# robotic-vision-lab/Learning-Implicitly-From-Spatial-Transformers-Network

Measured on AMD Instinct MI355X. Metric: SDF query-points/sec (B=8, N=20k, 224^2), higher is better.
Workload: dtype fp16

## Files before the change

learning-implicitly-from-spatial-transformers-network_amd/csrc/prep_kernels.hip:

```cpp
#include "list_common.h"
#include "gather_math.h"

namespace list {

constexpr int kResizeCg = 32;
constexpr int kResizeMaxMs = 320;

__global__ __launch_bounds__(256) void k_prep_img(ListMap2D m, int ms, int Ct, int coff, int f16,
                                                  void* __restrict__ out) {
  __shared__ float tile[kResizeMaxMs * (kResizeCg + 1)];
  const int b = blockIdx.x / ms;
  const int y = blockIdx.x - b * ms;
  const int c0 = blockIdx.y * kResizeCg;
  const int nc = min(kResizeCg, m.C - c0);

  const float sy = ms > 1 ? (float)(m.H - 1) / (float)(ms - 1) : 0.f;
  const float sx = ms > 1 ? (float)(m.W - 1) / (float)(ms - 1) : 0.f;
  const float fy = sy * (float)y;
  const int y0 = min((int)fy, m.H - 1);
  const int y1 = y0 + (y0 < m.H - 1 ? 1 : 0);
  const float wy1 = fy - (float)y0, wy0 = 1.f - wy1;
  const float* base = m.data + (int64_t)b * m.sb;

  for (int idx = threadIdx.x; idx < nc * ms; idx += 256) {
    const int cl = idx / ms;
    const int x = idx - cl * ms;
    const float fx = sx * (float)x;
    const int x0 = min((int)fx, m.W - 1);
    const int x1 = x0 + (x0 < m.W - 1 ? 1 : 0);
    const float wx1 = fx - (float)x0, wx0 = 1.f - wx1;
    const float* pc = base + (int64_t)(c0 + cl) * m.sc;
    const float v00 = pc[(int64_t)y0 * m.sh + (int64_t)x0 * m.sw];
// ... 457 lines not shown
    const uint2 lo = half4(make_float4(v[0], v[1], v[2], v[3])), hi = half4(make_float4(v[4], v[5], v[6], v[7]));
    *(uint4*)((unsigned short*)out + o) = make_uint4(lo.x, lo.y, hi.x, hi.y);
  } else {
    *(float4*)((float*)out + o) = make_float4(v[0], v[1], v[2], v[3]);
    *(float4*)((float*)out + o + 4) = make_float4(v[4], v[5], v[6], v[7]);
  }
}

hipError_t launch_img_level_rows(const ListMap2D* maps, void* const* outs, int n, int B, int f16, hipStream_t s) {
  if (n < 1 || n > LIST_N_IMG_LEVELS || B < 1) return hipErrorInvalidValue;
  LevelRowsArgs a;
  a.n = n; a.B = B;
  int64_t blocks = 0;
  for (int i = 0; i < n; ++i) {
    const ListMap2D& m = maps[i];
    if (m.C % 64 || m.H < 1 || m.W < 1) return hipErrorInvalidValue;
    a.m[i] = m; a.out[i] = outs[i]; a.blk_begin[i] = (int)blocks;
    blocks += (int64_t)B * ((m.H * m.W + 31) / 32) * (m.C / 64);
    if (blocks >= 2147483647LL) return hipErrorInvalidValue;
  }
  for (int i = n; i < LIST_N_IMG_LEVELS; ++i) { a.m[i] = maps[0]; a.out[i] = outs[0]; a.blk_begin[i] = (int)blocks; }
  a.blk_begin[LIST_N_IMG_LEVELS] = (int)blocks;
  if (f16) hipLaunchKernelGGL(k_img_level_rows<1>, dim3((unsigned)blocks), dim3(256), 0, s, a);
  else hipLaunchKernelGGL(k_img_level_rows<0>, dim3((unsigned)blocks), dim3(256), 0, s, a);
  return hipGetLastError();
}

constexpr int kProjPx = 64, kProjN = 256;
struct ProjLevelArgs {
  ListMap2D m[LIST_N_IMG_LEVELS]; const unsigned short* w[LIST_N_IMG_LEVELS]; unsigned short* out[LIST_N_IMG_LEVELS];
  int blk_begin[LIST_N_IMG_LEVELS + 1]; int n, B, H1, ldw;
};

__global__ __launch_bounds__(256) void k_proj_level_nchw(ProjLevelArgs a) {
  __shared__ uint4 As[2][kProjPx * 8];
  int r = 0;
#pragma unroll
  for (int i = 1; i < LIST_N_IMG_LEVELS; ++i)
    if (i < a.n && (int)blockIdx.x >= a.blk_begin[i]) r = i;
  const int l = a.n - 1 - r;
  const ListMap2D m = a.m[l];
  const int npx = m.H * m.W, pbs = (npx + kProjPx - 1) / kProjPx, nts = a.H1 / kProjN;
  int idx = (int)blockIdx.x - a.blk_begin[r];
  const int nt = idx % nts; idx /= nts;
  const int pb = idx % pbs;
  const int b = idx / pbs;
  const int p0 = pb * kProjPx, n0 = nt * kProjN;
  const int lane = threadIdx.x & 63, wave = threadIdx.x >> 6;
  const int col = lane & 15, ko = lane >> 4;
  const int px = min(p0 + lane, npx - 1);
  const int y = px / m.W, x = px - y * m.W;
  const float* src = m.data + (int64_t)b * m.sb + (int64_t)y * m.sh + (int64_t)x * m.sw + (int64_t)(16 * wave) * m.sc;
  const unsigned short* wrow = a.w[l] + (int64_t)(n0 + wave * 64 + col) * a.ldw + 8 * ko;
  const int nk = m.C / 64;
  float v[16];
  auto fetch = [&](int t) {
#pragma unroll
    for (int k = 0; k < 16; ++k) v[k] = src[(int64_t)(t * 64 + k) * m.sc];
  };
  f32x4v acc[4][4];
#pragma unroll
  for (int i = 0; i < 4; ++i)
#pragma unroll
    for (int j = 0; j < 4; ++j) acc[i][j] = (f32x4v){0.f, 0.f, 0.f, 0.f};
  f16x8 bw[2][4], bn[2][4];
  auto fetch_w = [&](int t, f16x8 (&d)[2][4]) {
#pragma unroll
    for (int ks = 0; ks < 2; ++ks)
#pragma unroll
      for (int j = 0; j < 4; ++j) d[ks][j] = *(const f16x8*)(wrow + (int64_t)(j * 16) * a.ldw + t * 64 + ks * 32);
  };
  fetch(0);
  fetch_w(0, bw);
#pragma unroll 1
  for (int t = 0; t < nk; ++t) {
    uint4* buf = As[t & 1];
#pragma unroll
    for (int o = 0; o < 2; ++o) {
      const uint2 lo = half4(make_float4(v[8 * o], v[8 * o + 1], v[8 * o + 2], v[8 * o + 3]));
      const uint2 hi = half4(make_float4(v[8 * o + 4], v[8 * o + 5], v[8 * o + 6], v[8 * o + 7]));
      buf[lane * 8 + ((2 * wave + o) ^ (lane & 7))] = make_uint4(lo.x, lo.y, hi.x, hi.y);
    }
    if (t + 1 < nk) { fetch(t + 1); fetch_w(t + 1, bn); }
    __syncthreads();
#pragma unroll
    for (int ks = 0; ks < 2; ++ks) {
      f16x8 fa[4];
#pragma unroll
      for (int i = 0; i < 4; ++i)
        fa[i] = __builtin_bit_cast(f16x8, buf[(i * 16 + col) * 8 + ((4 * ks + ko) ^ (col & 7))]);
#pragma unroll
      for (int i = 0; i < 4; ++i)
#pragma unroll
        for (int j = 0; j < 4; ++j) acc[i][j] = __builtin_amdgcn_mfma_f32_16x16x32_f16(bw[ks][j], fa[i], acc[i][j], 0, 0, 0);
    }
#pragma unroll
    for (int ks = 0; ks < 2; ++ks)
#pragma unroll
      for (int j = 0; j < 4; ++j) bw[ks][j] = bn[ks][j];
  }
#pragma unroll
  for (int i = 0; i < 4; ++i) {
    const int p = p0 + i * 16 + col;
    if (p >= npx) continue;
    unsigned short* o = a.out[l] + ((int64_t)b * npx + p) * a.H1 + n0 + wave * 64 + 4 * ko;
#pragma unroll
    for (int j = 0; j < 4; ++j)
      *(uint2*)(o + j * 16) = half4(make_float4(acc[i][j][0], acc[i][j][1], acc[i][j][2], acc[i][j][3]));
  }
}

hipError_t launch_proj_levels_nchw(const ListMap2D* maps, const void* const* w, void* const* outs, int n, int B, int H1,
                                   int ldw, hipStream_t s, int order) {
  if (n < 1 || n > LIST_N_IMG_LEVELS || B < 1 || H1 < kProjN || H1 % kProjN || ldw < 64 || ldw % 8) return hipErrorInvalidValue;
  ProjLevelArgs a;
  a.n = n; a.B = B; a.H1 = H1; a.ldw = ldw;
  int64_t blocks = 0;
  for (int r = 0; r < n; ++r) {
    const int i = n - 1 - r;
    const ListMap2D& m = maps[i];
    if (m.C < 64 || m.C % 64 || m.H < 1 || m.W < 1 || (reinterpret_cast<uintptr_t>(w[i]) & 15) ||
        (reinterpret_cast<uintptr_t>(outs[i]) & 7))
      return hipErrorInvalidValue;
    a.m[i] = m; a.w[i] = (const unsigned short*)w[i]; a.out[i] = (unsigned short*)outs[i]; a.blk_begin[r] = (int)blocks;
    blocks += (int64_t)B * ((m.H * m.W + kProjPx - 1) / kProjPx) * (H1 / kProjN);
    if (blocks >= 2147483647LL) return hipErrorInvalidValue;
  }
  for (int i = n; i < LIST_N_IMG_LEVELS; ++i) { a.m[i] = a.m[0]; a.w[i] = a.w[0]; a.out[i] = a.out[0]; a.blk_begin[i] = (int)blocks; }
  a.blk_begin[LIST_N_IMG_LEVELS] = (int)blocks;
  LIST_LAUNCH(k_proj_level_nchw, dim3((unsigned)blocks), dim3(256), 0, s, order, a);
  return hipGetLastError();
}

constexpr int kProjMaxSrc = LIST_N_IMG_LEVELS;
struct ProjSumArgs { ListMap2D src[kProjMaxSrc]; int n_src, B, ms, Ct, coff, H1, RY, nyt, nxt; };

template <int F16, int NL, int SRC16>
__global__ __launch_bounds__(kRowsPx * 8) void k_proj_resize_sum(ProjSumArgs a, void* __restrict__ out) {
  const int bid = xcd_contiguous_block(blockIdx.x, gridDim.x);
  const int cgroups = a.H1 / kRowsCg;
  int idx = bid;
  const int xt = idx % a.nxt; idx /= a.nxt;
  const int cg = idx % cgroups; idx /= cgroups;
  const int yt = idx % a.nyt;
  const int b = idx / a.nyt;
  const int ms = a.ms;
  const int q = threadIdx.x & 7, xi = threadIdx.x >> 3;
  const int xo = xt * kRowsPx + xi;
  const bool active = xo < ms;
  const int x = active ? xo : ms - 1;
  const int c = cg * kRowsCg + 8 * q;

  float top[NL][8], bot[NL][8];
  int row_top[NL], row_bot[NL];
  int64_t p0[NL], p1[NL];
// ... 40 lines not shown
    for (int k = 0; k < 8; ++k) o[k] = 0.f;
#pragma unroll
    for (int l = 0; l < NL; ++l) {
      const int H = a.src[l].H;
      const float fy = sy[l] * (float)y;
      const int y0 = min((int)fy, H - 1);
      const int y1 = y0 + (y0 < H - 1 ? 1 : 0);
      const float wy1 = fy - (float)y0, wy0 = 1.f - wy1;
      if (y0 != row_top[l]) {
        if (y0 == row_bot[l]) {
#pragma unroll
          for (int k = 0; k < 8; ++k) top[l][k] = bot[l][k];
        } else {
          hrow(l, y0, top[l]);
        }
        row_top[l] = y0;
      }
      if (y1 != row_bot[l]) {
        if (y1 == row_top[l]) {
#pragma unroll
          for (int k = 0; k < 8; ++k) bot[l][k] = top[l][k];
        } else {
          hrow(l, y1, bot[l]);
        }
        row_bot[l] = y1;
      }
#pragma unroll
      for (int k = 0; k < 8; ++k) o[k] += top[l][k] * wy0 + bot[l][k] * wy1;
    }
    if (!active) continue;
    if (F16) {
      const uint2 lo = half4(make_float4(o[0], o[1], o[2], o[3]));
      const uint2 hi = half4(make_float4(o[4], o[5], o[6], o[7]));
      *(uint4*)((unsigned short*)out + oi) = make_uint4(lo.x, lo.y, hi.x, hi.y);
    } else {
      *(float4*)((float*)out + oi) = make_float4(o[0], o[1], o[2], o[3]);
      *(float4*)((float*)out + oi + 4) = make_float4(o[4], o[5], o[6], o[7]);
    }
  }
}

hipError_t launch_proj_resize_sum(const ListMap2D* src, int n_src, int B, int map_size, int Ct, int coff, int f16,
                                  void* out, hipStream_t s, int src_f16) {
  if (n_src < 1 || n_src > kProjMaxSrc || map_size < 2 || B < 1) return hipErrorInvalidValue;
  ProjSumArgs a;
  a.n_src = n_src; a.B = B; a.ms = map_size; a.Ct = Ct; a.coff = coff; a.H1 = src[0].C;
  if (a.H1 % kRowsCg || coff % 8 || Ct % 8) return hipErrorInvalidValue;
  float sy_max = 0.f;
  for (int l = 0; l < n_src; ++l) {
    const ListMap2D& m = src[l];
    const int al = src_f16 ? 8 : 4;
    if (m.C != a.H1 || m.sc != 1 || (m.sw % al) || (m.sh % al) || (m.sb % al) || (reinterpret_cast<uintptr_t>(m.data) & 15))
      return hipErrorInvalidValue;
    a.src[l] = m;
    const float sy = (float)(m.H - 1) / (float)(map_size - 1);
    sy_max = sy > sy_max ? sy : sy_max;
  }
  for (int l = n_src; l < kProjMaxSrc; ++l) a.src[l] = src[0];
  int ry = (int)(6.6f / (sy_max > 0.05f ? sy_max : 0.05f) + 0.5f);
  a.RY = ry < 2 ? 2 : (ry > kRowsRyMax ? kRowsRyMax : ry);
  a.nyt = (map_size + a.RY - 1) / a.RY;
  a.nxt = (map_size + kRowsPx - 1) / kRowsPx;
  const int64_t wgs = (int64_t)B * a.nyt * (a.H1 / kRowsCg) * a.nxt;
  if (wgs <= 0 || wgs >= 2147483647LL) return hipErrorInvalidValue;
  const dim3 grid((unsigned)wgs), block(kRowsPx * 8);
#define LIST_PROJ_SUM(NL)                                                                      \
  case NL:                                                                                     \
// ... 304 lines not shown
```

learning-implicitly-from-spatial-transformers-network_amd/csrc/gemm_kernels.hip:

```cpp
#include <type_traits>

#include "list_common.h"
#include "mfma_common.h"
#include "point_math.h"
#include "gather_math.h"

namespace list {

constexpr int BM = 256, BN = 256;
constexpr int kLdsBytes = 131072;
constexpr int kProjRecBytes = BM * (int)sizeof(RowProjRec);

template <int TERMS> struct Pipe {
  static constexpr int kPlanes = TERMS == 3 ? 4 : 2;
  static constexpr int BK = TERMS == 3 ? 32 : 64;
  static constexpr int kRowBytes = BK * 2;
  static constexpr int kPlaneBytes = BM * kRowBytes;
  static constexpr int kStageBytes = kPlanes * kPlaneBytes;
  static constexpr int kStages = kLdsBytes / kStageBytes;
  static constexpr int kAhead = kStages - 1;
  static constexpr int kRowsPerPiece = 1024 / kRowBytes;
  static constexpr int kPiecesPerWave = BM / kRowsPerPiece / 8;
  static constexpr int kLoadsPerStage = kPiecesPerWave * kPlanes;
  static constexpr int kWOff = (TERMS == 3 ? 2 : 1) * kPlaneBytes;
  __device__ static __forceinline__ int swz(int row) {
    return kRowBytes == 64 ? ((row >> 2) & 3) : ((row >> 1) & 7);
  }
};

template <int TERMS>
__device__ __forceinline__ void stage_tiles(const GemmParams& p, char* sbase, int m0, int n0,
                                            int kbyte, int wave, int lane) {
// ... 726 lines not shown
        ah[i] = *(const bf16x8*)(cur + a_row_off + i * 16 * P::kRowBytes + coff);
        if (TERMS == 3)
          al[i] = *(const bf16x8*)(cur + P::kPlaneBytes + a_row_off + i * 16 * P::kRowBytes + coff);
      }
#pragma unroll
      for (int j = 0; j < 4; ++j) {
        wh[j] = *(const bf16x8*)(cur + P::kWOff + w_row_off + j * 16 * P::kRowBytes + coff);
        if (TERMS == 3)
          wl[j] = *(const bf16x8*)(cur + P::kWOff + P::kPlaneBytes + w_row_off + j * 16 * P::kRowBytes + coff);
      }
#pragma unroll
      for (int i = 0; i < 8; ++i)
#pragma unroll
        for (int j = 0; j < 4; ++j) {
          if (TERMS == 3) {
            acc[i][j] = mfma16<0>(al[i], wh[j], acc[i][j]);
            acc[i][j] = mfma16<0>(ah[i], wl[j], acc[i][j]);
          }
          acc[i][j] = mfma16<FP16>(ah[i], wh[j], acc[i][j]);
        }
    }
  }

  gemm_epilogue16<EPI, FP16>(p, acc, smem, m0, n0, wm, wn, wave, lane);
}

struct TailParams {
  GemmParams fc1;
  const char* w2; const float* b2;
  const float* w3; const float* b3; float* sdf; const int* order; int n_valid;
};
constexpr int kTailLds = 163840;

__global__ __launch_bounds__(512, 2) void k_mlp_tail_f16(TailParams tp) {
  using P = Pipe<1>;
  __shared__ __attribute__((aligned(16))) char smem[kTailLds];
  const int lane = threadIdx.x & 63;
  const int wave = __builtin_amdgcn_readfirstlane(threadIdx.x >> 6);
  const int m0 = xcd_contiguous_block(blockIdx.x, gridDim.x) * BM;
  const int col = lane & 15, q = lane >> 4;
  const int fswz = P::swz(col);
  const GemmParams& p = tp.fc1;

  auto w2_base = [&](int kt) -> char* { return smem + (kt == 0 ? 131072 : (kt - 1) * 32768); };
  auto stage_w2 = [&](int kt) {
#pragma unroll
    for (int r = 0; r < 4; ++r) {
      const int piece = 4 * wave + r;
      const int row = piece * 8 + lane / 8;
      const int chunk = (lane % 8) ^ P::swz(row);
      glds16(tp.w2 + (int64_t)row * 512 + kt * 128 + chunk * 16, w2_base(kt) + piece * 1024);
    }
  };
  stage_w2(0);

  f32x4v acc[16][2];
#pragma unroll
  for (int i = 0; i < 16; ++i)
#pragma unroll
    for (int j = 0; j < 2; ++j)
#pragma unroll
      for (int e = 0; e < 4; ++e) acc[i][j][e] = 0.f;
  const int h_row_off = (wave * 32 + col) * P::kRowBytes;
  const int wrow_e = 8 * (col >> 2) + (col & 3), wrow_o = wrow_e + 4;
  const int wswz_e = P::swz(wrow_e), wswz_o = P::swz(wrow_o);
  const int nk = p.K / P::BK;
  stage_tiles<1>(p, smem, m0, 0, 0, wave, lane);
  for (int t = 0; t < nk; ++t) {
    wait_vmcnt<0>();
    __builtin_amdgcn_s_barrier();
    if (t + 1 < nk) stage_tiles<1>(p, smem + ((t + 1) & 1) * P::kStageBytes, m0, 0, (t + 1) * P::kRowBytes, wave, lane);
    const char* cur = smem + (t & 1) * P::kStageBytes;
#pragma unroll
    for (int s2 = 0; s2 < 2; ++s2) {
      const int coff = ((4 * s2 + q) ^ fswz) << 4;
      bf16x8 hf[2];
#pragma unroll
      for (int rt = 0; rt < 2; ++rt) hf[rt] = *(const bf16x8*)(cur + h_row_off + rt * 16 * P::kRowBytes + coff);
#pragma unroll
      for (int nt = 0; nt < 16; ++nt) {
        const int wrow = 32 * (nt >> 1) + ((nt & 1) ? wrow_o : wrow_e);
        const bf16x8 wf = *(const bf16x8*)(cur + P::kWOff + wrow * P::kRowBytes + (((4 * s2 + q) ^ ((nt & 1) ? wswz_o : wswz_e)) << 4));
#pragma unroll
        for (int rt = 0; rt < 2; ++rt) acc[nt][rt] = mfma16<1>(wf, hf[rt], acc[nt][rt]);
      }
    }
  }
  float4 b1v[16];
#pragma unroll
  for (int nt = 0; nt < 16; ++nt) b1v[nt] = *(const float4*)(p.bias + 32 * (nt >> 1) + 8 * q + 4 * (nt & 1));
  __syncthreads();
  stage_w2(1); stage_w2(2); stage_w2(3);
  uint2 h2[16][2];
#pragma unroll
  for (int nt = 0; nt < 16; ++nt) {
    const float bb[4] = {b1v[nt].x, b1v[nt].y, b1v[nt].z, b1v[nt].w};
#pragma unroll
    for (int rt = 0; rt < 2; ++rt) {
      float v[4];
#pragma unroll
      for (int e = 0; e < 4; ++e) v[e] = relu_nan(acc[nt][rt][e] + bb[e]);
      h2[nt][rt] = make_uint2(f2h2(v[0], v[1]), f2h2(v[2], v[3]));
    }
  }
  f32x4v acc2[16][2];
#pragma unroll
  for (int i = 0; i < 16; ++i)
#pragma unroll
    for (int j = 0; j < 2; ++j)
#pragma unroll
      for (int e = 0; e < 4; ++e) acc2[i][j][e] = 0.f;
#pragma unroll
  for (int ks = 0; ks < 8; ++ks) {
    if (ks == 2) { wait_vmcnt<8>(); __builtin_amdgcn_s_barrier(); }
    if (ks == 4) { wait_vmcnt<4>(); __builtin_amdgcn_s_barrier(); }
    if (ks == 6) { wait_vmcnt<0>(); __builtin_amdgcn_s_barrier(); }
    const char* wt = w2_base(ks >> 1);
    const int coff = ((4 * (ks & 1) + q) ^ fswz) << 4;
    bf16x8 hb[2];
#pragma unroll
    for (int rt = 0; rt < 2; ++rt)
      hb[rt] = __builtin_bit_cast(bf16x8, make_uint4(h2[2 * ks][rt].x, h2[2 * ks][rt].y, h2[2 * ks + 1][rt].x, h2[2 * ks + 1][rt].y));
#pragma unroll
    for (int mt = 0; mt < 16; ++mt) {
      const bf16x8 wf = *(const bf16x8*)(wt + (mt * 16 + col) * P::kRowBytes + coff);
#pragma unroll
      for (int rt = 0; rt < 2; ++rt) acc2[mt][rt] = mfma16<1>(wf, hb[rt], acc2[mt][rt]);
    }
  }
  float grp[2][4];
#pragma unroll
  for (int gq = 0; gq < 4; ++gq) {
    float sc[2][4];
#pragma unroll
    for (int rt = 0; rt < 2; ++rt)
#pragma unroll
      for (int e = 0; e < 4; ++e) sc[rt][e] = 0.f;
#pragma unroll
    for (int j = 0; j < 4; ++j) {
      const int mt = 4 * gq + j;
      const float4 b2v = *(const float4*)(tp.b2 + 16 * mt + 4 * q), w3v = *(const float4*)(tp.w3 + 16 * mt + 4 * q);
      const float bb[4] = {b2v.x, b2v.y, b2v.z, b2v.w}, ww[4] = {w3v.x, w3v.y, w3v.z, w3v.w};
#pragma unroll
      for (int rt = 0; rt < 2; ++rt)
#pragma unroll
        for (int e = 0; e < 4; ++e) sc[rt][e] += relu_nan(acc2[mt][rt][e] + bb[e]) * ww[e];
    }
#pragma unroll
    for (int rt = 0; rt < 2; ++rt) {
#pragma unroll
      for (int e = 0; e < 4; ++e) {
        sc[rt][e] += __shfl_xor(sc[rt][e], 32);
        sc[rt][e] += __shfl_xor(sc[rt][e], 16);
      }
      const float a0 = sc[rt][0] + sc[rt][2], a1 = sc[rt][1] + sc[rt][3];
      grp[rt][gq] = a0 + a1;
    }
  }
#pragma unroll
  for (int rt = 0; rt < 2; ++rt) {
    const int row = m0 + wave * 32 + rt * 16 + col;
    if (q == 0 && row < tp.n_valid)
      tp.sdf[tp.order ? tp.order[row] : row] = ((grp[rt][0] + grp[rt][1]) + (grp[rt][2] + grp[rt][3])) + tp.b3[0];
  }
}

hipError_t launch_mlp_tail(const GemmParams& fc1, const char* w2, const float* b2, const float* w3, const float* b3,
                           float* sdf, const int* order, int n_valid, hipStream_t s) {
  if (fc1.fmt != FMT_FP16 || fc1.N != BN || fc1.M % BM || fc1.K % 64 || fc1.K < 64 || !fc1.bias) return hipErrorInvalidValue;
  TailParams tp;
  tp.fc1 = fc1; tp.w2 = w2; tp.b2 = b2; tp.w3 = w3; tp.b3 = b3; tp.sdf = sdf; tp.order = order; tp.n_valid = n_valid;
  hipLaunchKernelGGL(k_mlp_tail_f16, dim3(fc1.M / BM), dim3(512), 0, s, tp);
  return hipGetLastError();
}

template <int TERMS, int EPI, int FP16>
static hipError_t launch_one(const GemmParams& p, hipStream_t s) {
  const int ntiles = (p.M / BM) * (p.N / BN);
  if constexpr (FP16 == 0 && (EPI == EPI_RELU_SPLIT || EPI == EPI_F32 || EPI == EPI_DX)) {
    if (p.x3i) {
      if constexpr (TERMS == 3) hipLaunchKernelGGL((k_gemm_nt_pp<EPI, 0, true, 3>), dim3(ntiles), dim3(512), 0, s, p);
      else hipLaunchKernelGGL((k_gemm_nt_pp<EPI, 0, true, 1>), dim3(ntiles), dim3(512), 0, s, p);
      return hipGetLastError();
    }
  }
  if (p.x3i) return hipErrorInvalidValue;
  const bool need_pp = p.lda || p.ldw || p.a_rows || p.rowvec || p.k_gap || p.n_groups;
  if constexpr (EPI == EPI_RELU_DOT)
    hipLaunchKernelGGL((k_gemm_nt16<TERMS, EPI, FP16>), dim3(ntiles), dim3(512), 0, s, p);
  else {
    if constexpr (TERMS == 1 && (EPI == EPI_RELU_SPLIT || EPI == EPI_F32 || EPI == EPI_DX || EPI == EPI_MASK_SPLIT)) {
      if (p.K >= kPpMinK || need_pp) {
        if (!p.plain_loop) hipLaunchKernelGGL((k_gemm_nt_pp<EPI, FP16, true>), dim3(ntiles), dim3(512), 0, s, p);
        else hipLaunchKernelGGL((k_gemm_nt16<TERMS, EPI, FP16>), dim3(ntiles), dim3(512), 0, s, p);
        return hipGetLastError();
      }
    }
    if (need_pp) return hipErrorInvalidValue;
    if constexpr (TERMS == 3 && (EPI == EPI_RELU_SPLIT || EPI == EPI_F32)) {
      if (p.K >= 1024) {
        hipLaunchKernelGGL((k_gemm_nt16<TERMS, EPI, FP16>), dim3(ntiles), dim3(512), 0, s, p);
        return hipGetLastError();
      }
    }
    if constexpr (EPI == EPI_DX || EPI == EPI_MASK_SPLIT) {
// ... 57 lines not shown
```

Before: 90.41 million.

## Cut proj kernel registers, stage output through LDS, nontemporal resize stores

The projection GEMM kernel drops the double-buffered weight registers. It now prefetches next-tile weights per k-slice after the MFMAs, with a sched barrier, and sets launch bounds to request 3 waves per SIMD for higher occupancy. The last tile is peeled through a compile-time flag so the hot loop carries no branch. Output tiles are staged through a larger swizzled LDS buffer so each row is written with coalesced 16-byte stores, which requires 16-byte output alignment. Separately, fp16 stores in the resize-sum kernel become nontemporal, trading cache residency for write bandwidth if that output is read soon after.

```diff
diff --git a/learning-implicitly-from-spatial-transformers-network_amd/csrc/prep_kernels.hip b/learning-implicitly-from-spatial-transformers-network_amd/csrc/prep_kernels.hip
--- a/learning-implicitly-from-spatial-transformers-network_amd/csrc/prep_kernels.hip
+++ b/learning-implicitly-from-spatial-transformers-network_amd/csrc/prep_kernels.hip
@@ -1,3 +1,4 @@
+#include <type_traits>
 #include "list_common.h"
 #include "gather_math.h"
 
@@ -521,8 +522,8 @@
   int blk_begin[LIST_N_IMG_LEVELS + 1]; int n, B, H1, ldw;
 };
 
-__global__ __launch_bounds__(256) void k_proj_level_nchw(ProjLevelArgs a) {
-  __shared__ uint4 As[2][kProjPx * 8];
+__global__ __launch_bounds__(256, 3) void k_proj_level_nchw(ProjLevelArgs a) {
+  __shared__ uint4 As[kProjPx * 32];
   int r = 0;
 #pragma unroll
   for (int i = 1; i < LIST_N_IMG_LEVELS; ++i)
@@ -552,25 +553,23 @@
   for (int i = 0; i < 4; ++i)
 #pragma unroll
     for (int j = 0; j < 4; ++j) acc[i][j] = (f32x4v){0.f, 0.f, 0.f, 0.f};
-  f16x8 bw[2][4], bn[2][4];
-  auto fetch_w = [&](int t, f16x8 (&d)[2][4]) {
-#pragma unroll
-    for (int ks = 0; ks < 2; ++ks)
-#pragma unroll
-      for (int j = 0; j < 4; ++j) d[ks][j] = *(const f16x8*)(wrow + (int64_t)(j * 16) * a.ldw + t * 64 + ks * 32);
+  f16x8 bw[2][4];
+  auto fetch_w = [&](int t, int ks) {
+#pragma unroll
+    for (int j = 0; j < 4; ++j) bw[ks][j] = *(const f16x8*)(wrow + (int64_t)(j * 16) * a.ldw + t * 64 + ks * 32);
   };
   fetch(0);
-  fetch_w(0, bw);
-#pragma unroll 1
-  for (int t = 0; t < nk; ++t) {
-    uint4* buf = As[t & 1];
+  fetch_w(0, 0);
+  fetch_w(0, 1);
+  auto k_tile = [&](int t, auto more) {
+    uint4* buf = As + (t & 1) * (kProjPx * 8);
 #pragma unroll
     for (int o = 0; o < 2; ++o) {
       const uint2 lo = half4(make_float4(v[8 * o], v[8 * o + 1], v[8 * o + 2], v[8 * o + 3]));
       const uint2 hi = half4(make_float4(v[8 * o + 4], v[8 * o + 5], v[8 * o + 6], v[8 * o + 7]));
       buf[lane * 8 + ((2 * wave + o) ^ (lane & 7))] = make_uint4(lo.x, lo.y, hi.x, hi.y);
     }
-    if (t + 1 < nk) { fetch(t + 1); fetch_w(t + 1, bn); }
+    if (more.value) fetch(t + 1);
     __syncthreads();
 #pragma unroll
     for (int ks = 0; ks < 2; ++ks) {
@@ -582,20 +581,32 @@
       for (int i = 0; i < 4; ++i)
 #pragma unroll
         for (int j = 0; j < 4; ++j) acc[i][j] = __builtin_amdgcn_mfma_f32_16x16x32_f16(bw[ks][j], fa[i], acc[i][j], 0, 0, 0);
-    }
-#pragma unroll
-    for (int ks = 0; ks < 2; ++ks)
-#pragma unroll
-      for (int j = 0; j < 4; ++j) bw[ks][j] = bn[ks][j];
-  }
+      if (more.value) {
+        fetch_w(t + 1, ks);
+        if (ks == 0) __builtin_amdgcn_sched_barrier(0);
+      }
+    }
+  };
+#pragma unroll 1
+  for (int t = 0; t < nk - 1; ++t) k_tile(t, std::true_type());
+  k_tile(nk - 1, std::false_type());
+  __syncthreads();
+  uint2* img = (uint2*)As;
 #pragma unroll
   for (int i = 0; i < 4; ++i) {
-    const int p = p0 + i * 16 + col;
-    if (p >= npx) continue;
-    unsigned short* o = a.out[l] + ((int64_t)b * npx + p) * a.H1 + n0 + wave * 64 + 4 * ko;
+    const int p = i * 16 + col;
 #pragma unroll
     for (int j = 0; j < 4; ++j)
-      *(uint2*)(o + j * 16) = half4(make_float4(acc[i][j][0], acc[i][j][1], acc[i][j][2], acc[i][j][3]));
+      img[(p * 32 + ((8 * wave + 2 * j + (ko >> 1)) ^ (col & 7))) * 2 + (ko & 1)] =
+          half4(make_float4(acc[i][j][0], acc[i][j][1], acc[i][j][2], acc[i][j][3]));
+  }
+  __syncthreads();
+  const int q = threadIdx.x & 31, pr = threadIdx.x >> 5;
+  unsigned short* o = a.out[l] + ((int64_t)b * npx + p0) * a.H1 + n0 + 8 * q;
+#pragma unroll
+  for (int i = 0; i < kProjPx / 8; ++i) {
+    const int p = i * 8 + pr;
+    if (p0 + p < npx) *(uint4*)(o + (int64_t)p * a.H1) = As[p * 32 + (q ^ (p & 7))];
   }
 }
 
@@ -609,7 +620,7 @@
     const int i = n - 1 - r;
     const ListMap2D& m = maps[i];
     if (m.C < 64 || m.C % 64 || m.H < 1 || m.W < 1 || (reinterpret_cast<uintptr_t>(w[i]) & 15) ||
-        (reinterpret_cast<uintptr_t>(outs[i]) & 7))
+        (reinterpret_cast<uintptr_t>(outs[i]) & 15))
       return hipErrorInvalidValue;
     a.m[i] = m; a.w[i] = (const unsigned short*)w[i]; a.out[i] = (unsigned short*)outs[i]; a.blk_begin[r] = (int)blocks;
     blocks += (int64_t)B * ((m.H * m.W + kProjPx - 1) / kProjPx) * (H1 / kProjN);
@@ -716,7 +727,9 @@
     if (F16) {
       const uint2 lo = half4(make_float4(o[0], o[1], o[2], o[3]));
       const uint2 hi = half4(make_float4(o[4], o[5], o[6], o[7]));
-      *(uint4*)((unsigned short*)out + oi) = make_uint4(lo.x, lo.y, hi.x, hi.y);
+      __builtin_nontemporal_store((f32x4){__builtin_bit_cast(float, lo.x), __builtin_bit_cast(float, lo.y),
+                                          __builtin_bit_cast(float, hi.x), __builtin_bit_cast(float, hi.y)},
+                                  (f32x4*)((unsigned short*)out + oi));
     } else {
       *(float4*)((float*)out + oi) = make_float4(o[0], o[1], o[2], o[3]);
       *(float4*)((float*)out + oi + 4) = make_float4(o[4], o[5], o[6], o[7]);
```

Result: no change. 89.77 million (median of 2 runs) (-0.7%).

## Add persistent weight-stationary MLP tail kernel with pipelined row blocks

Applied to the files above, without the earlier changes.

Adds a persistent kernel for the fc1->fc2->fc3 SDF tail when K is 512. It launches one workgroup per CU, keeps W1 and W2 fragments resident in registers and streams 32-row activation blocks through a triple-buffered LDS ring with async global-to-LDS loads. The final dot-product reduction is split across wave halves and deferred to the next iteration so it overlaps the next block's matrix work. This removes repeated weight loads per 256-row tile, at the cost of very high register pressure, smaller MFMA tiles and an environment-variable switch for fallback.

```diff
diff --git a/learning-implicitly-from-spatial-transformers-network_amd/csrc/gemm_kernels.hip b/learning-implicitly-from-spatial-transformers-network_amd/csrc/gemm_kernels.hip
--- a/learning-implicitly-from-spatial-transformers-network_amd/csrc/gemm_kernels.hip
+++ b/learning-implicitly-from-spatial-transformers-network_amd/csrc/gemm_kernels.hip
@@ -1,3 +1,6 @@
+#include <algorithm>
+#include <atomic>
+#include <cstdlib>
 #include <type_traits>
 
 #include "list_common.h"
@@ -923,11 +926,288 @@
   }
 }
 
+constexpr int kWsRows = 32;
+constexpr int kWsH1Ld = 1024 + 32, kWsH1Bytes = kWsRows * kWsH1Ld;
+constexpr int kWsH2Ld = 512 + 32, kWsH2Bytes = kWsRows * kWsH2Ld;
+constexpr int kWsH2Off = 3 * kWsH1Bytes;
+constexpr int kWsPartOff = kWsH2Off + kWsH2Bytes, kWsPartBytes = 4 * 8 * 64 * 4;
+constexpr int kWsTermOff = kWsPartOff + 2 * kWsPartBytes, kWsTermBytes = 4 * 16 * 64 * 4;
+constexpr int kWsGrpOff = kWsTermOff + kWsTermBytes, kWsGrpBytes = 4 * kWsRows * 4;
+constexpr int kWsConstOff = kWsGrpOff + 2 * kWsGrpBytes;
+constexpr int kWsOrdOff = kWsConstOff + 3 * 1024;
+constexpr int kWsLds = kWsOrdOff + 4 * 256;
+constexpr int kWsK = 512;
+static_assert(kWsLds <= kTailLds, "one workgroup per CU");
+
+__device__ __forceinline__ void lds_store_asm(unsigned addr, float v) {
+  asm volatile("ds_write_b32 %0, %1" ::"v"(addr), "v"(v) : "memory");
+}
+__device__ __forceinline__ void lds_store_asm(unsigned addr, uint2 v) {
+  const unsigned long long d = (unsigned long long)v.x | ((unsigned long long)v.y << 32);
+  asm volatile("ds_write_b64 %0, %1" ::"v"(addr), "v"(d) : "memory");
+}
+
+template <bool ORDER>
+__global__ __launch_bounds__(512, 2) void k_mlp_tail_ws_f16(TailParams tp) {
+  constexpr int P = ORDER ? 5 : 4;
+  __shared__ __attribute__((aligned(16))) char smem[kWsLds];
+  const GemmParams& p = tp.fc1;
+  const int nblocks = p.M / kWsRows;
+  const int first = blockIdx.x, stride = gridDim.x;
+  if (first >= nblocks) return;
+  const int n = (nblocks - first + stride - 1) / stride;
+  const int lane = threadIdx.x & 63;
+  const int wave = __builtin_amdgcn_readfirstlane(threadIdx.x >> 6);
+  const int col = lane & 15, q = lane >> 4;
+  const bool odd = wave >> 2;
+  const int gq = wave & 3;
+  const int c2 = 64 * gq + 32 * (wave >> 2);
+  const unsigned lds0 = (unsigned)(size_t)(__attribute__((address_space(3))) char*)smem;
+
+  float* cst = (float*)(smem + kWsConstOff);
+  if (threadIdx.x < 256) {
+    cst[threadIdx.x] = p.bias[threadIdx.x];
+    cst[256 + threadIdx.x] = tp.b2[threadIdx.x];
+    cst[512 + threadIdx.x] = tp.w3[threadIdx.x];
+  }
+  const float b3v = tp.b3[0];
+
+  bf16x8 w1f[2][16], w2f[2][8];
+#pragma unroll
+  for (int nt = 0; nt < 2; ++nt)
+#pragma unroll
+    for (int ks = 0; ks < 16; ++ks)
+      w1f[nt][ks] = *(const bf16x8*)(p.w_hi + (int64_t)(32 * wave + 16 * nt + col) * (kWsK * 2) + 64 * ks + 16 * q);
+#pragma unroll
+  for (int nt = 0; nt < 2; ++nt)
+#pragma unroll
+    for (int ks = 0; ks < 8; ++ks)
+      w2f[nt][ks] = *(const bf16x8*)(tp.w2 + (c2 + 16 * nt + col) * 512 + 64 * ks + 16 * q);
+
+  const unsigned src_lo = (unsigned)lane * 16;
+  auto stage_h1 = [&](int blk, int slot, int slot4) {
+#pragma unroll
+    for (int r = 0; r < 4; ++r) {
+      const int row = wave + 8 * r;
+      const char* rowp = p.a_hi + ((int64_t)blk * kWsRows + row) * (kWsK * 2);
+      glds16(rowp + src_lo, smem + slot * kWsH1Bytes + row * kWsH1Ld);
+    }
+    if constexpr (ORDER) {
+      const int row = max(min(blk * kWsRows + (lane & 31), tp.n_valid - 1), 0);
+      __builtin_amdgcn_global_load_lds((const __attribute__((address_space(1))) void*)(tp.order + row),
+                                       (__attribute__((address_space(3))) void*)(smem + kWsOrdOff + (slot4 & 3) * 256), 4, 0, 0);
+    }
+  };
+  stage_h1(first, 0, 0);
+  if (n > 1) stage_h1(first + stride, 1, 1);
+
+  auto lane_now = [&]() { int l = lane; asm volatile("" : "+v"(l)); return l; };
+
+  auto fc_out_terms = [&](const f32x4v (&a)[2], int j, int q, float (&t)[2][4]) {
+    const float* cb = cst + 256 + c2 + 16 * j + 4 * q;
+    const float bb[4] = {cb[0], cb[1], cb[2], cb[3]}, ww[4] = {cb[256], cb[257], cb[258], cb[259]};
+#pragma unroll
+    for (int rt = 0; rt < 2; ++rt)
+#pragma unroll
+      for (int e = 0; e < 4; ++e) t[rt][e] = relu_nan(a[rt][e] + bb[e]) * ww[e];
+  };
+  auto fc_out_group = [&](int par) {
+    const int lane = lane_now(), col = lane & 15, q = lane >> 4;
+    const float* pr = (const float*)(smem + kWsPartOff + par * kWsPartBytes) + gq * 512 + lane;
+    float sc[2][4];
+#pragma unroll
+    for (int rt = 0; rt < 2; ++rt)
+#pragma unroll
+      for (int e = 0; e < 4; ++e) sc[rt][e] = pr[(rt * 4 + e) * 64];
+    const float* tr = (const float*)(smem + kWsTermOff) + gq * 16 * 64 + lane;
+#pragma unroll
+    for (int j = 0; j < 2; ++j)
+#pragma unroll
+      for (int rt = 0; rt < 2; ++rt)
+#pragma unroll
+        for (int e = 0; e < 4; ++e) sc[rt][e] += tr[(j * 8 + rt * 4 + e) * 64];
+    const unsigned gw = lds0 + kWsGrpOff + par * kWsGrpBytes + (gq * kWsRows + col) * 4;
+#pragma unroll
+    for (int rt = 0; rt < 2; ++rt) {
+#pragma unroll
+      for (int e = 0; e < 4; ++e) {
+        sc[rt][e] += __shfl_xor(sc[rt][e], 32);
+        sc[rt][e] += __shfl_xor(sc[rt][e], 16);
+      }
+      const float a0 = sc[rt][0] + sc[rt][2], a1 = sc[rt][1] + sc[rt][3];
+      if (q == 0) lds_store_asm(gw + rt * 64, a0 + a1);
+    }
+  };
+  auto fc_out_store = [&](int blk, int par, int slot4) {
+    const int lane = lane_now();
+    if (wave == 0 && lane < kWsRows) {
+      const float* g = (const float*)(smem + kWsGrpOff + par * kWsGrpBytes) + lane;
+      const int row = blk * kWsRows + lane;
+      int to = row;
+      if constexpr (ORDER) to = *((const int*)(smem + kWsOrdOff + (slot4 & 3) * 256) + lane);
+      if (row < tp.n_valid) tp.sdf[to] = ((g[0] + g[kWsRows]) + (g[2 * kWsRows] + g[3 * kWsRows])) + b3v;
+    }
+  };
+
+  int slot = 0;
+  for (int i = 0; i < n; ++i) {
+    const int blk = first + i * stride, par = i & 1;
+    if (i + 1 < n) wait_vmcnt<P>(); else wait_vmcnt<0>();
+    asm volatile("s_waitcnt lgkmcnt(0)" ::: "memory");
+    __builtin_amdgcn_s_barrier();
+    asm volatile("" ::: "memory");
+    if (i + 2 < n) stage_h1(blk + 2 * stride, slot >= 1 ? slot - 1 : 2, i + 2);
+    if (odd && i > 0) fc_out_group(par ^ 1);
+
+    f32x4v acc[2][2];
+#pragma unroll
+    for (int nt = 0; nt < 2; ++nt)
+#pragma unroll
+      for (int rt = 0; rt < 2; ++rt)
+#pragma unroll
+        for (int e = 0; e < 4; ++e) acc[nt][rt][e] = 0.f;
+    {
+      const int l = lane_now();
+      const char* cur = smem + slot * kWsH1Bytes + (l & 15) * kWsH1Ld + 16 * (l >> 4);
+      bf16x8 hf[3][2];
+#pragma unroll
+      for (int ks = 0; ks < 2; ++ks)
+#pragma unroll
+        for (int rt = 0; rt < 2; ++rt) hf[ks][rt] = *(const bf16x8*)(cur + (64 * ks + rt * 16 * kWsH1Ld));
+#pragma unroll
+      for (int ks = 0; ks < 16; ++ks) {
+        if (ks + 2 < 16) {
+#pragma unroll
+          for (int rt = 0; rt < 2; ++rt) hf[(ks + 2) % 3][rt] = *(const bf16x8*)(cur + (64 * (ks + 2) + rt * 16 * kWsH1Ld));
+        }
+        __builtin_amdgcn_sched_barrier(0);
+#pragma unroll
+        for (int nt = 0; nt < 2; ++nt)
+#pragma unroll
+          for (int rt = 0; rt < 2; ++rt) acc[nt][rt] = mfma16<1>(w1f[nt][ks], hf[ks % 3][rt], acc[nt][rt]);
+        __builtin_amdgcn_sched_barrier(0);
+      }
+    }
+    const int lane = lane_now(), col = lane & 15, q = lane >> 4;
+    const unsigned h2_st = lds0 + kWsH2Off + col * kWsH2Ld + 64 * wave + 8 * q;
+#pragma unroll
+    for (int nt = 0; nt < 2; ++nt) {
+      const float* cb = cst + 32 * wave + 16 * nt + 4 * q;
+      const float bb[4] = {cb[0], cb[1], cb[2], cb[3]};
+#pragma unroll
+      for (int rt = 0; rt < 2; ++rt) {
+        float v[4];
+#pragma unroll
+        for (int e = 0; e < 4; ++e) v[e] = relu_nan(acc[nt][rt][e] + bb[e]);
+        lds_store_asm(h2_st + (32 * nt + rt * 16 * kWsH2Ld), make_uint2(f2h2(v[0], v[1]), f2h2(v[2], v[3])));
+      }
+    }
+    asm volatile("s_waitcnt lgkmcnt(0)" ::: "memory");
+    __builtin_amdgcn_s_barrier();
+    asm volatile("" ::: "memory");
+
+    f32x4v acc2[2][2];
+#pragma unroll
+    for (int nt = 0; nt < 2; ++nt)
+#pragma unroll
+      for (int rt = 0; rt < 2; ++rt)
+#pragma unroll
+        for (int e = 0; e < 4; ++e) acc2[nt][rt][e] = 0.f;
+    {
+      const char* h2r = smem + kWsH2Off + col * kWsH2Ld + 16 * q;
+      bf16x8 hb[3][2];
+#pragma unroll
+      for (int ks = 0; ks < 2; ++ks)
+#pragma unroll
+        for (int rt = 0; rt < 2; ++rt) hb[ks][rt] = *(const bf16x8*)(h2r + (64 * ks + rt * 16 * kWsH2Ld));
+#pragma unroll
+      for (int ks = 0; ks < 8; ++ks) {
+        if (ks + 2 < 8) {
+#pragma unroll
+          for (int rt = 0; rt < 2; ++rt) hb[(ks + 2) % 3][rt] = *(const bf16x8*)(h2r + (64 * (ks + 2) + rt * 16 * kWsH2Ld));
+        }
+        __builtin_amdgcn_sched_barrier(0);
+#pragma unroll
+        for (int nt = 0; nt < 2; ++nt)
+#pragma unroll
+          for (int rt = 0; rt < 2; ++rt) acc2[nt][rt] = mfma16<1>(w2f[nt][ks], hb[ks % 3][rt], acc2[nt][rt]);
+        __builtin_amdgcn_sched_barrier(0);
+      }
+    }
+    if (odd) {
+      const unsigned tw = lds0 + kWsTermOff + (gq * 16 * 64 + lane) * 4;
+#pragma unroll
+      for (int j = 0; j < 2; ++j) {
+        float t[2][4];
+        fc_out_terms(acc2[j], j, q, t);
+#pragma unroll
+        for (int rt = 0; rt < 2; ++rt)
+#pragma unroll
+          for (int e = 0; e < 4; ++e) lds_store_asm(tw + (j * 8 + rt * 4 + e) * 256, t[rt][e]);
+      }
+    } else {
+      float sc[2][4];
+#pragma unroll
+      for (int rt = 0; rt < 2; ++rt)
+#pragma unroll
+        for (int e = 0; e < 4; ++e) sc[rt][e] = 0.f;
+#pragma unroll
+      for (int j = 0; j < 2; ++j) {
+        float t[2][4];
+        fc_out_terms(acc2[j], j, q, t);
+#pragma unroll
+        for (int rt = 0; rt < 2; ++rt)
+#pragma unroll
+          for (int e = 0; e < 4; ++e) sc[rt][e] += t[rt][e];
+      }
+      const unsigned pw = lds0 + kWsPartOff + par * kWsPartBytes + (gq * 512 + lane) * 4;
+#pragma unroll
+      for (int rt = 0; rt < 2; ++rt)
+#pragma unroll
+        for (int e = 0; e < 4; ++e) lds_store_asm(pw + (rt * 4 + e) * 256, sc[rt][e]);
+    }
+    if (i > 0) fc_out_store(blk - stride, par ^ 1, i - 1);
+    slot = slot == 2 ? 0 : slot + 1;
+  }
+  const int lpar = (n - 1) & 1;
+  asm volatile("s_waitcnt lgkmcnt(0)" ::: "memory");
+  __builtin_amdgcn_s_barrier();
+  asm volatile("" ::: "memory");
+  if (odd) fc_out_group(lpar);
+  asm volatile("s_waitcnt lgkmcnt(0)" ::: "memory");
+  __builtin_amdgcn_s_barrier();
+  asm volatile("" ::: "memory");
+  fc_out_store(first + (n - 1) * stride, lpar, n - 1);
+}
+
+static int device_cu_count() {
+  static std::atomic<int> cus[64];
+  int dev = 0;
+  if (hipGetDevice(&dev) != hipSuccess || dev < 0 || dev >= 64) return 0;
+  int c = cus[dev].load(std::memory_order_relaxed);
+  if (c == 0) {
+    if (hipDeviceGetAttribute(&c, hipDeviceAttributeMultiprocessorCount, dev) != hipSuccess || c <= 0) return 0;
+    cus[dev].store(c, std::memory_order_relaxed);
+  }
+  return c;
+}
+
 hipError_t launch_mlp_tail(const GemmParams& fc1, const char* w2, const float* b2, const float* w3, const float* b3,
                            float* sdf, const int* order, int n_valid, hipStream_t s) {
   if (fc1.fmt != FMT_FP16 || fc1.N != BN || fc1.M % BM || fc1.K % 64 || fc1.K < 64 || !fc1.bias) return hipErrorInvalidValue;
   TailParams tp;
   tp.fc1 = fc1; tp.w2 = w2; tp.b2 = b2; tp.w3 = w3; tp.b3 = b3; tp.sdf = sdf; tp.order = order; tp.n_valid = n_valid;
+  if (fc1.K == kWsK) {
+    const char* e = getenv("LIST_TAIL_WS");
+    if (!(e && e[0] == '0' && e[1] == 0)) {
+      const int cus = device_cu_count();
+      if (cus <= 0) return hipErrorInvalidDevice;
+      const dim3 grid(std::min(cus, fc1.M / kWsRows));
+      if (order) hipLaunchKernelGGL(k_mlp_tail_ws_f16<true>, grid, dim3(512), 0, s, tp);
+      else hipLaunchKernelGGL(k_mlp_tail_ws_f16<false>, grid, dim3(512), 0, s, tp);
+      return hipGetLastError();
+    }
+  }
   hipLaunchKernelGGL(k_mlp_tail_f16, dim3(fc1.M / BM), dim3(512), 0, s, tp);
   return hipGetLastError();
 }
```

Measured after the change: 90.18 million before, 90.86 million after (median of 6 runs). Within noise of the previous version (+0.8%).

## Make MLP tail kernel persistent with cross-tile prefetch through a rotating LDS plane ring

Applied to the files above, without the earlier changes.

The fused fc1→fc2→fc3 tail kernel now launches at most one block per CU, and each block loops over a contiguous range of 256-row tiles. LDS is reorganised into three H planes and two W planes used as a ring, so fc1 K-tiles are prefetched two steps ahead. The fc2 weight planes and the next tile's first fc1 loads are issued during the current tile's fc2 phase, hiding the per-tile pipeline fill and launch tail. The code also makes global source addresses wave-uniform via readfirstlane and caches the CU count on the host. The cost is much more intricate vmcnt and barrier accounting and fewer resident blocks to hide latency.

```diff
diff --git a/learning-implicitly-from-spatial-transformers-network_amd/csrc/gemm_kernels.hip b/learning-implicitly-from-spatial-transformers-network_amd/csrc/gemm_kernels.hip
--- a/learning-implicitly-from-spatial-transformers-network_amd/csrc/gemm_kernels.hip
+++ b/learning-implicitly-from-spatial-transformers-network_amd/csrc/gemm_kernels.hip
@@ -1,3 +1,4 @@
+#include <atomic>
 #include <type_traits>
 
 #include "list_common.h"
@@ -790,65 +791,109 @@
 };
 constexpr int kTailLds = 163840;
 
+__device__ __forceinline__ const char* uniform_ptr(const char* ptr) {
+  const uint64_t v = (uint64_t)ptr;
+  const unsigned lo = __builtin_amdgcn_readfirstlane((unsigned)v), hi = __builtin_amdgcn_readfirstlane((unsigned)(v >> 32));
+  return (const char*)(((uint64_t)hi << 32) | lo);
+}
+
 __global__ __launch_bounds__(512, 2) void k_mlp_tail_f16(TailParams tp) {
   using P = Pipe<1>;
   __shared__ __attribute__((aligned(16))) char smem[kTailLds];
+  const int wave = __builtin_amdgcn_readfirstlane(threadIdx.x >> 6);
+  const GemmParams& p = tp.fc1;
+  const int nk = p.K / P::BK;
+
+  const int ntiles = p.M / BM;
+  const int run = xcd_contiguous_block(blockIdx.x, gridDim.x);
+  const int tile0 = (int)((int64_t)run * ntiles / gridDim.x);
+  const int tile_end = (int)((int64_t)(run + 1) * ntiles / gridDim.x);
+
+  auto hplane = [&](int i) -> char* { return smem + i * P::kPlaneBytes; };
+  auto wplane = [&](int i) -> char* { return smem + (3 + i) * P::kPlaneBytes; };
+  const unsigned pitch1 = 2 * p.K, pitch2 = 512;
+  auto h1_src = [&](int tl, int t) { return p.a_hi + (int64_t)tl * BM * (2 * p.K) + t * P::kRowBytes; };
+  auto w1_src = [&](int t) { return p.w_hi + t * P::kRowBytes; };
+  auto w2_src = [&](int kt) { return tp.w2 + kt * P::kRowBytes; };
+  auto next3 = [](int i) { return i == 2 ? 0 : i + 1; };
+
   const int lane = threadIdx.x & 63;
-  const int wave = __builtin_amdgcn_readfirstlane(threadIdx.x >> 6);
-  const int m0 = xcd_contiguous_block(blockIdx.x, gridDim.x) * BM;
   const int col = lane & 15, q = lane >> 4;
   const int fswz = P::swz(col);
-  const GemmParams& p = tp.fc1;
-
-  auto w2_base = [&](int kt) -> char* { return smem + (kt == 0 ? 131072 : (kt - 1) * 32768); };
-  auto stage_w2 = [&](int kt) {
-#pragma unroll
-    for (int r = 0; r < 4; ++r) {
-      const int piece = 4 * wave + r;
-      const int row = piece * 8 + lane / 8;
-      const int chunk = (lane % 8) ^ P::swz(row);
-      glds16(tp.w2 + (int64_t)row * 512 + kt * 128 + chunk * 16, w2_base(kt) + piece * 1024);
-    }
+  unsigned off1[2], off2[2];
+#pragma unroll
+  for (int o = 0; o < 2; ++o) {
+    const int chunk = (lane % 8) ^ (4 * o + (lane >> 4));
+    off1[o] = (lane / 8) * pitch1 + chunk * 16;
+    off2[o] = (lane / 8) * pitch2 + chunk * 16;
+  }
+  auto stage_plane = [&](const char* src, unsigned pitch, const unsigned (&off)[2], char* dst) {
+#pragma unroll
+    for (int r = 0; r < 4; ++r)
+      glds16(uniform_ptr(src + (int64_t)(32 * wave + 8 * r) * pitch) + off[r & 1], dst + (4 * wave + r) * 1024);
   };
-  stage_w2(0);
-
-  f32x4v acc[16][2];
-#pragma unroll
-  for (int i = 0; i < 16; ++i)
-#pragma unroll
-    for (int j = 0; j < 2; ++j)
-#pragma unroll
-      for (int e = 0; e < 4; ++e) acc[i][j][e] = 0.f;
   const int h_row_off = (wave * 32 + col) * P::kRowBytes;
   const int wrow_e = 8 * (col >> 2) + (col & 3), wrow_o = wrow_e + 4;
   const int wswz_e = P::swz(wrow_e), wswz_o = P::swz(wrow_o);
-  const int nk = p.K / P::BK;
-  stage_tiles<1>(p, smem, m0, 0, 0, wave, lane);
-  for (int t = 0; t < nk; ++t) {
-    wait_vmcnt<0>();
+
+  int tile = tile0;
+  int hb = 0, wb = 0;
+  stage_plane(h1_src(tile, 0), pitch1, off1, hplane(0));
+  stage_plane(w1_src(0), pitch1, off1, wplane(0));
+  if (nk > 1) stage_plane(h1_src(tile, 1), pitch1, off1, hplane(1));
+  else stage_plane(w2_src(0), pitch2, off2, hplane(1));
+
+  auto row_tile = [&](auto next_c) {
+  constexpr bool has_next = decltype(next_c)::value;
+  const int m0 = tile * BM;
+  f32x4v acc[16][2];
+#pragma unroll
+  for (int i = 0; i < 16; ++i)
+#pragma unroll
+    for (int j = 0; j < 2; ++j)
+#pragma unroll
+      for (int e = 0; e < 4; ++e) acc[i][j][e] = 0.f;
+  int hs = hb, ws = wb;
+  auto k_tile = [&](const char* src_w, unsigned pitch_w, const unsigned (&off_w)[2], const char* src_h, unsigned pitch_h,
+                    const unsigned (&off_h)[2]) {
+    wait_vmcnt<4>();
     __builtin_amdgcn_s_barrier();
-    if (t + 1 < nk) stage_tiles<1>(p, smem + ((t + 1) & 1) * P::kStageBytes, m0, 0, (t + 1) * P::kRowBytes, wave, lane);
-    const char* cur = smem + (t & 1) * P::kStageBytes;
+    stage_plane(src_w, pitch_w, off_w, wplane(ws ^ 1));
+    stage_plane(src_h, pitch_h, off_h, hplane(next3(next3(hs))));
+    const char* ch = hplane(hs);
+    const char* cw = wplane(ws);
 #pragma unroll
     for (int s2 = 0; s2 < 2; ++s2) {
       const int coff = ((4 * s2 + q) ^ fswz) << 4;
       bf16x8 hf[2];
 #pragma unroll
-      for (int rt = 0; rt < 2; ++rt) hf[rt] = *(const bf16x8*)(cur + h_row_off + rt * 16 * P::kRowBytes + coff);
+      for (int rt = 0; rt < 2; ++rt) hf[rt] = *(const bf16x8*)(ch + h_row_off + rt * 16 * P::kRowBytes + coff);
 #pragma unroll
       for (int nt = 0; nt < 16; ++nt) {
         const int wrow = 32 * (nt >> 1) + ((nt & 1) ? wrow_o : wrow_e);
-        const bf16x8 wf = *(const bf16x8*)(cur + P::kWOff + wrow * P::kRowBytes + (((4 * s2 + q) ^ ((nt & 1) ? wswz_o : wswz_e)) << 4));
+        const bf16x8 wf = *(const bf16x8*)(cw + wrow * P::kRowBytes + (((4 * s2 + q) ^ ((nt & 1) ? wswz_o : wswz_e)) << 4));
 #pragma unroll
         for (int rt = 0; rt < 2; ++rt) acc[nt][rt] = mfma16<1>(wf, hf[rt], acc[nt][rt]);
       }
     }
-  }
+    hs = next3(hs); ws ^= 1;
+  };
+  for (int t = 0; t < nk; ++t) {
+    const bool w_in = t + 1 < nk, h_in = t + 2 < nk;
+    const unsigned off_w[2] = {w_in ? off1[0] : off2[0], w_in ? off1[1] : off2[1]};
+    const unsigned off_h[2] = {h_in ? off1[0] : off2[0], h_in ? off1[1] : off2[1]};
+    k_tile(w_in ? w1_src(t + 1) : w2_src(1), w_in ? pitch1 : pitch2, off_w,
+           h_in ? h1_src(tile, t + 2) : w2_src(t + 2 == nk ? 0 : 2), h_in ? pitch1 : pitch2, off_h);
+  }
+  const int hs1 = next3(hs), hs2 = next3(hs1);
   float4 b1v[16];
 #pragma unroll
-  for (int nt = 0; nt < 16; ++nt) b1v[nt] = *(const float4*)(p.bias + 32 * (nt >> 1) + 8 * q + 4 * (nt & 1));
-  __syncthreads();
-  stage_w2(1); stage_w2(2); stage_w2(3);
+  for (int nt = 0; nt < 16; ++nt) b1v[nt] = *(const float4*)((const char*)p.bias + (unsigned)(32 * q) + 128 * (nt >> 1) + 16 * (nt & 1));
+  wait_vmcnt<0>();
+  __builtin_amdgcn_s_barrier();
+  stage_plane(w2_src(3), pitch2, off2, wplane(ws ^ 1));
+  if (has_next) stage_plane(h1_src(tile + 1, 0), pitch1, off1, hplane(hs2));
+  const char* const w2_plane[4] = {hplane(hs), wplane(ws), hplane(hs1), wplane(ws ^ 1)};
   uint2 h2[16][2];
 #pragma unroll
   for (int nt = 0; nt < 16; ++nt) {
@@ -870,10 +915,19 @@
       for (int e = 0; e < 4; ++e) acc2[i][j][e] = 0.f;
 #pragma unroll
   for (int ks = 0; ks < 8; ++ks) {
-    if (ks == 2) { wait_vmcnt<8>(); __builtin_amdgcn_s_barrier(); }
-    if (ks == 4) { wait_vmcnt<4>(); __builtin_amdgcn_s_barrier(); }
-    if (ks == 6) { wait_vmcnt<0>(); __builtin_amdgcn_s_barrier(); }
-    const char* wt = w2_base(ks >> 1);
+    if (ks == 4 && has_next) {
+      __builtin_amdgcn_s_barrier();
+      const bool h_in = nk > 1;
+      stage_plane(w1_src(0), pitch1, off1, wplane(ws));
+      const unsigned off_h[2] = {h_in ? off1[0] : off2[0], h_in ? off1[1] : off2[1]};
+      stage_plane(h_in ? h1_src(tile + 1, 1) : w2_src(0), h_in ? pitch1 : pitch2, off_h, hplane(hs));
+    }
+    if (ks == 6) {
+      if (has_next) wait_vmcnt<12>(); else wait_vmcnt<0>();
+      __builtin_amdgcn_s_barrier();
+    }
+    __builtin_amdgcn_sched_barrier(0);
+    const char* wt = w2_plane[ks >> 1];
     const int coff = ((4 * (ks & 1) + q) ^ fswz) << 4;
     bf16x8 hb[2];
 #pragma unroll
@@ -897,7 +951,8 @@
 #pragma unroll
     for (int j = 0; j < 4; ++j) {
       const int mt = 4 * gq + j;
-      const float4 b2v = *(const float4*)(tp.b2 + 16 * mt + 4 * q), w3v = *(const float4*)(tp.w3 + 16 * mt + 4 * q);
+      const float4 b2v = *(const float4*)((const char*)tp.b2 + (unsigned)(16 * q) + 64 * mt);
+      const float4 w3v = *(const float4*)((const char*)tp.w3 + (unsigned)(16 * q) + 64 * mt);
       const float bb[4] = {b2v.x, b2v.y, b2v.z, b2v.w}, ww[4] = {w3v.x, w3v.y, w3v.z, w3v.w};
 #pragma unroll
       for (int rt = 0; rt < 2; ++rt)
@@ -921,6 +976,10 @@
     if (q == 0 && row < tp.n_valid)
       tp.sdf[tp.order ? tp.order[row] : row] = ((grp[rt][0] + grp[rt][1]) + (grp[rt][2] + grp[rt][3])) + tp.b3[0];
   }
+  ++tile; hb = hs2; wb = ws;
+  };
+  while (tile + 1 < tile_end) row_tile(std::true_type());
+  row_tile(std::false_type());
 }
 
 hipError_t launch_mlp_tail(const GemmParams& fc1, const char* w2, const float* b2, const float* w3, const float* b3,
@@ -928,7 +987,19 @@
   if (fc1.fmt != FMT_FP16 || fc1.N != BN || fc1.M % BM || fc1.K % 64 || fc1.K < 64 || !fc1.bias) return hipErrorInvalidValue;
   TailParams tp;
   tp.fc1 = fc1; tp.w2 = w2; tp.b2 = b2; tp.w3 = w3; tp.b3 = b3; tp.sdf = sdf; tp.order = order; tp.n_valid = n_valid;
-  hipLaunchKernelGGL(k_mlp_tail_f16, dim3(fc1.M / BM), dim3(512), 0, s, tp);
+  constexpr int kMaxDevices = 64;
+  static std::atomic<int> cu_count[kMaxDevices];
+  int dev = 0;
+  hipError_t e = hipGetDevice(&dev);
+  if (e != hipSuccess) return e;
+  int cus = dev < kMaxDevices ? cu_count[dev].load(std::memory_order_relaxed) : 0;
+  if (cus <= 0) {
+    e = hipDeviceGetAttribute(&cus, hipDeviceAttributeMultiprocessorCount, dev);
+    if (e != hipSuccess || cus <= 0) return e != hipSuccess ? e : hipErrorInvalidDevice;
+    if (dev < kMaxDevices) cu_count[dev].store(cus, std::memory_order_relaxed);
+  }
+  const int ntiles = fc1.M / BM;
+  hipLaunchKernelGGL(k_mlp_tail_f16, dim3(ntiles < cus ? ntiles : cus), dim3(512), 0, s, tp);
   return hipGetLastError();
 }
 
```

Result: no change. 90.86 million before, 91.24 million after, median of 6 (+0.4%).
